# Circuitscape/Circuitscape.jl

Hardware: NVIDIA H100
Metric: pair_solves_per_sec (higher is better)
Workload: dtype f64

## Files before the change

circuitscape_b200/csrc/cs_b200.cu:

```cuda
#include "../../include/cs_b200.h"

#include <cuda_runtime.h>

#include <algorithm>
#include <chrono>
#include <cmath>
#include <cstdarg>
#include <cstdio>
#include <cstdlib>
#include <cstring>
#include <limits>
#include <string>
#include <type_traits>
#include <vector>

#include "amg_host.hpp"
#include "win_host.hpp"
#include "kernels.cuh"
#include "raster_assembly.cuh"
#include "setup_device.hpp"

using namespace csb;

namespace {
// ... 659 lines not shown
  if (rc) return rc;
  return cs_b200_reset_currents(h);
}

template <typename T>
int build_operators(cs_b200_handle* h, const csb_dev::HostPattern& hp, csb_dev::SeedJob* job,
                    const csb_dev::DeviceSeed* dseed) {
  int rc = CS_B200_OK;
  k_dinv<T><<<std::min<int64_t>((h->n_pad + 255) / 256, 4096), 256, 0, h->stream>>>(
      (int)h->n, (int)h->n_pad, h->d_rowptr, h->d_colidx, (const T*)h->d_vals, (T*)h->d_dinv);
  const bool want_win = h->opts.window >= 0 && (h->opts.window > 0 || h->n >= 20000) && (win_mask() & 1);
  const bool want_amg = h->opts.precond == CS_B200_PRECOND_AMG;
  Tick tick;
  if (want_win || h->opts.stencil > 0) {
    rc = device_stencil<T>(h, h->A0);
    if (!rc && !h->A0.dia && want_win) rc = device_windows<T>(h, h->A0, h->n_pad, (const T*)h->d_dinv);
    if (rc) { csb_dev::seed_discard(job); return rc; }
    tick(h->A0.dia ? "finest operator: stencil form" : "finest operator: windows");
  }
  if (want_amg) {
    rc = setup_amg_device<T>(h, hp, job, dseed);
    if (rc) return rc;
    if (h->amg && h->A0.dia && !h->P2) {
      const size_t pe = (size_t)h->n_pad * h->ktmax * sizeof(T);
      cudaError_t e = cudaMalloc(&h->P2, pe);
      if (e == cudaSuccess) e = cudaMemsetAsync(h->P2, 0, pe, h->stream);
      if (e != cudaSuccess) return set_err(h, CS_B200_ERR_CUDA, "CUDA error %s (second p panel)", cudaGetErrorString(e));
    }
  } else {
    csb_dev::seed_discard(job);
  }
  Tick tick1;
  csb_dev::trim_pool(h->device);
  tick1("scratch pool released");
  return CS_B200_OK;
}

int common_create(cs_b200_handle* h, const cs_b200_opts* opts) {
  if (opts) h->opts = *opts;
  if (h->opts.panel_width == 0) h->opts.panel_width = 8;
  if (h->opts.check_every <= 0) h->opts.check_every = 16;
  if (h->opts.resid_gate <= 0) h->opts.resid_gate = 1e-4;
  if (h->opts.use_graph == 0) h->opts.use_graph = 1;
  const int pw = h->opts.panel_width;
  if (pw != 1 && pw != 2 && pw != 4 && pw != 8)
    return set_err(h, CS_B200_ERR_ARG, "panel_width must be 1, 2, 4 or 8 (got %d)", pw);
  h->ktmax = pw;
  if (h->opts.precond != CS_B200_PRECOND_JACOBI && h->opts.precond != CS_B200_PRECOND_AMG)
    return set_err(h, CS_B200_ERR_UNSUPPORTED, "unknown preconditioner %d", h->opts.precond);
  int ndev = 0;
  cudaError_t e = cudaGetDeviceCount(&ndev);
  if (e != cudaSuccess || ndev == 0)
    return set_err(h, CS_B200_ERR_CUDA,
                   "no CUDA device available (%s): libcsb200 has no CPU fallback",
                   cudaGetErrorString(e));
  if (h->device < 0 || h->device >= ndev)
    return set_err(h, CS_B200_ERR_ARG, "device %d out of range (0..%d)", h->device, ndev - 1);
  CK(h, cudaSetDevice(h->device));
  cudaDeviceProp prop;
  CK(h, cudaGetDeviceProperties(&prop, h->device));
  h->num_sms = prop.multiProcessorCount;
  h->grid_spmm = h->num_sms * 8;
  h->grid_ew = h->num_sms * 4;
  CK(h, cudaStreamCreateWithFlags(&h->stream, cudaStreamNonBlocking));
  CK(h, cudaEventCreate(&h->ev0));
  CK(h, cudaEventCreate(&h->ev1));
  CK(h, cudaEventCreate(&h->ev2));
  CK(h, cudaEventCreate(&h->ev3));
  h->n_pad = (h->n + 3) / 4 * 4;
  return CS_B200_OK;
}

template <typename I>
void narrow_indices(const I* src, int64_t count, int base, std::vector<int>& dst) {
  dst.resize(count);
  for (int64_t i = 0; i < count; ++i) dst[i] = (int)(src[i] - base);
}

template <typename T>
CsrDev<T> view(const DevCsr& m) {
  return CsrDev<T>{m.rowptr, m.colidx, (const T*)m.vals, m.bstart, m.nblocks, m.nrows};
}

template <typename T, int KT, int MODE>
void launch_spmm_on(cs_b200_handle* h, const DevCsr& m, const T* X, T* Y, const T* B, const T* dinv,
                    double omega, bool timed) {
  const int grid = std::max(1, std::min(h->grid_spmm, m.nblocks));
  cudaEvent_t e0 = nullptr, e1 = nullptr;
  const bool prof = h->profile && timed;
  if (prof) {
    if (h->prof_used + 2 > h->prof_ev.size()) {
      for (int i = 0; i < 2; ++i) { cudaEvent_t e; cudaEventCreate(&e); h->prof_ev.push_back(e); }
    }
    e0 = h->prof_ev[h->prof_used++];
    e1 = h->prof_ev[h->prof_used++];
    double bytes = (double)m.nnz * (sizeof(T) + 4) + (double)(m.nrows + 1) * 4 +
                   2.0 * (double)m.nrows * KT * sizeof(T);
    if (MODE == SP_RESNORM || MODE == SP_RES || MODE == SP_JACOBI || MODE == SP_JACOBI_DOT)
      bytes += (double)m.nrows * KT * sizeof(T);
    if (MODE == SP_JACOBI || MODE == SP_JACOBI_DOT) bytes += (double)m.nrows * sizeof(T);
    h->prof_bytes += bytes;
    h->prof_slot.push_back(2 * MODE + (sizeof(T) == 4 ? 1 : 0));
    h->prof_pair_bytes.push_back(bytes);
    cudaEventRecord(e0, h->stream);
  }
  const SpmmEpi<T> ep{B, dinv, (T)omega, h->d_ctl, h->d_partials};
  if (m.dia && MODE != SP_ADD) {
    if constexpr (MODE != SP_ADD) {
      const DiaDev<T> a{(const T*)m.dia, m.dia_ld, m.nrows, m.dia_nr};
      constexpr int V16 = 16 / (int)sizeof(T);
      constexpr int CGn = KT / (KT < V16 ? KT : V16);
      const int rpp = NT / CGn;
      const long long ntiles = (long long)((m.dia_nr + rpp - 1) / rpp) *
                               ((((long long)m.nrows + m.dia_nr - 1) / m.dia_nr + ST_TC - 1) / ST_TC);
      const int sg = (int)std::max<long long>(1, std::min<long long>(h->grid_spmm, ntiles));
      k_stencil<T, KT, MODE><<<sg, NT, 0, h->stream>>>(a, X, Y, ep);
    }
  } else if (m.win_meta) {
    const WinCsr<T> w{m.win_meta, m.blob, m.has_dinv, m.rowptr, m.colidx, (const T*)m.vals, m.win_nblocks};
    if (m.lpr == 4) {
      constexpr int SMEM = WinSmem2<T, KT, MODE, true>::TOTAL;
      constexpr int SB = WinMap<T, KT, true>::SB;
      const int wg = std::max(1, std::min(h->num_sms, (m.win_nblocks + SB - 1) / SB));
      static bool once[64] = {};
      bool& set = once[h->device & 63];
      if (!set) { cudaFuncSetAttribute(k_spmm_win<T, KT, MODE, true>, cudaFuncAttributeMaxDynamicSharedMemorySize, SMEM); set = true; }
      k_spmm_win<T, KT, MODE, true><<<wg, WTT, SMEM, h->stream>>>(w, X, Y, ep);
    } else {
      constexpr int SMEM = WinSmem2<T, KT, MODE, false>::TOTAL;
      constexpr int SB = WinMap<T, KT, false>::SB;
      const int wg = std::max(1, std::min(h->num_sms, (m.win_nblocks + SB - 1) / SB));
      static bool once[64] = {};
      bool& set = once[h->device & 63];
      if (!set) { cudaFuncSetAttribute(k_spmm_win<T, KT, MODE, false>, cudaFuncAttributeMaxDynamicSharedMemorySize, SMEM); set = true; }
      k_spmm_win<T, KT, MODE, false><<<wg, WTT, SMEM, h->stream>>>(w, X, Y, ep);
    }
  } else if (m.lpr == 4 && KT * 4 <= 32) {
    k_spmm<T, KT, MODE, (KT * 4 <= 32 ? 4 : 1)><<<grid, NT, 0, h->stream>>>(view<T>(m), X, Y, ep);
  } else {
    k_spmm<T, KT, MODE, 1><<<grid, NT, 0, h->stream>>>(view<T>(m), X, Y, ep);
  }
  if (prof) cudaEventRecord(e1, h->stream);
  h->stats.kernel_launches++;
  if (timed) h->stats.spmm_launches++;
}

template <typename T, int KT, int MODE>
void launch_spmm(cs_b200_handle* h, const T* X, T* Y, const T* B) {
  launch_spmm_on<T, KT, MODE>(h, h->A0, X, Y, B, (const T*)h->d_dinv, 0.0, true);
}

void harvest_profile(cs_b200_handle* h) {
  for (size_t i = 0; i + 1 < h->prof_used; i += 2) {
    float ms = 0;
    if (cudaEventElapsedTime(&ms, h->prof_ev[i], h->prof_ev[i + 1]) == cudaSuccess) {
      h->prof_ms += ms;
      h->prof_launches++;
      if (i / 2 < h->prof_slot.size()) {
        const int sl = h->prof_slot[i / 2];
        h->prof_slot_ms[sl] += ms;
        h->prof_slot_bytes[sl] += h->prof_pair_bytes[i / 2];
        h->prof_slot_launches[sl]++;
      }
    }
  }
  h->prof_used = 0;
  h->prof_slot.clear();
  h->prof_pair_bytes.clear();
}

template <typename T, int KT>
int ew_grid(cs_b200_handle* h) {
  const size_t nelem = (size_t)h->n_pad * KT;
  const size_t per = (size_t)NT * Vec<T>::N;
  return (int)std::min<size_t>(h->grid_ew, (nelem + per - 1) / per);
}

template <typename T, int KT>
int ew_grid_n(cs_b200_handle* h, int64_t n_pad) {
  const size_t nelem = (size_t)n_pad * KT;
  const size_t per = (size_t)NT * Vec<T>::N;
  return (int)std::max<size_t>(1, std::min<size_t>(h->grid_ew, (nelem + per - 1) / per));
}

inline bool implicit_x0(const DevLevel& L) {
  static const bool off = std::getenv("CS_B200_NO_IMPLICIT_X0") != nullptr || std::getenv("CS_B200_NO_FUSED_PROLONG") != nullptr;
  return L.A.dia != nullptr && !off;
}

template <typename T, int KT>
void launch_stencil_res0(cs_b200_handle* h, DevLevel& L, const T* B, T* Tout, bool timed) {
  const DevCsr& m = L.A;
  const DiaDev<T> a{(const T*)m.dia, m.dia_ld, m.nrows, m.dia_nr};
  const SpmmEpi<T> ep{B, (const T*)L.dinv, (T)L.omega, h->d_ctl, h->d_partials};
  constexpr int V16 = 16 / (int)sizeof(T);
  constexpr int CGn = KT / (KT < V16 ? KT : V16);
  const int rpp = NT / CGn;
  const long long ntiles = (long long)((m.dia_nr + rpp - 1) / rpp) *
                           ((((long long)m.nrows + m.dia_nr - 1) / m.dia_nr + ST_TC - 1) / ST_TC);
  const int sg = (int)std::max<long long>(1, std::min<long long>(h->grid_spmm, ntiles));
  cudaEvent_t e0 = nullptr, e1 = nullptr;
  const bool prof = h->profile && timed;
  if (prof) {
    if (h->prof_used + 2 > h->prof_ev.size())
      for (int i = 0; i < 2; ++i) { cudaEvent_t e; cudaEventCreate(&e); h->prof_ev.push_back(e); }
    e0 = h->prof_ev[h->prof_used++];
    e1 = h->prof_ev[h->prof_used++];
    const double fb = (double)m.nnz * (sizeof(T) + 4) + (double)(m.nrows + 1) * 4 + 3.0 * (double)m.nrows * KT * sizeof(T);
    h->prof_bytes += fb;
    h->prof_slot.push_back(2 * (int)SP_RES + (sizeof(T) == 4 ? 1 : 0));
    h->prof_pair_bytes.push_back(fb);
    cudaEventRecord(e0, h->stream);
  }
  k_stencil<T, KT, SP_RES0><<<sg, NT, 0, h->stream>>>(a, nullptr, Tout, ep);
  if (prof) cudaEventRecord(e1, h->stream);
  h->stats.kernel_launches++;
  if (timed) h->stats.spmm_launches++;
}

template <typename T, int KT, int MODE>
void launch_prolong_jacobi(cs_b200_handle* h, DevLevel& L, const T* Yc, const T* X0, T* Yout, const T* B, bool timed) {
  const DevCsr& m = L.A;
  const DiaDev<T> a{(const T*)m.dia, m.dia_ld, m.nrows, m.dia_nr};
  const CsrP<T> p{L.P.rowptr, L.P.colidx, (const T*)L.P.vals, L.P.ell_col, (const T*)L.P.ell_val, L.P.ell_ld};
  const SpmmEpi<T> ep{B, (const T*)L.dinv, (T)L.omega, h->d_ctl, h->d_partials};
  using S = PjShape<T, KT>;
  constexpr int SMEM = S::SMEM;
  constexpr int MINB = sizeof(T) == 4 ? PJ_MINB_F32 : PJ_MINB_F64;
  static_assert(SMEM <= 48 * 1024, "the strip buffers fit the default dynamic shared memory");
  int occ = 0;
  cudaOccupancyMaxActiveBlocksPerMultiprocessor(&occ, k_stencil_prolong_jacobi<T, KT, MODE, MINB>, NT, SMEM);
  occ = std::max(1, occ);
  const long long nsteps = (long long)((m.dia_nr + S::RPS - 1) / S::RPS) *
                           (((long long)m.nrows + m.dia_nr - 1) / m.dia_nr);
  const int grid = (int)std::max<long long>(1, std::min<long long>(std::min(h->grid_spmm, h->num_sms * occ), nsteps));
  cudaEvent_t e0 = nullptr, e1 = nullptr;
  const bool prof = h->profile && timed;
  if (prof) {
    if (h->prof_used + 2 > h->prof_ev.size())
      for (int i = 0; i < 2; ++i) { cudaEvent_t e; cudaEventCreate(&e); h->prof_ev.push_back(e); }
    e0 = h->prof_ev[h->prof_used++];
    e1 = h->prof_ev[h->prof_used++];
    const double fb = (double)m.nnz * (sizeof(T) + 4) + (double)(m.nrows + 1) * 4 + 3.0 * (double)m.nrows * KT * sizeof(T) +
                      (double)m.nrows * sizeof(T) + (double)L.P.nnz * (sizeof(T) + 4) + (double)(m.nrows + 1) * 4 +
                      2.0 * (double)m.nrows * KT * sizeof(T);
    h->prof_bytes += fb;
    h->prof_slot.push_back(2 * 7 + (sizeof(T) == 4 ? 1 : 0));
    h->prof_pair_bytes.push_back(fb);
    cudaEventRecord(e0, h->stream);
  }
  k_stencil_prolong_jacobi<T, KT, MODE, MINB><<<grid, NT, SMEM, h->stream>>>(a, p, Yc, X0, Yout, ep);
  if (prof) cudaEventRecord(e1, h->stream);
  h->stats.kernel_launches++;
  if (timed) h->stats.spmm_launches++;
}

struct VcBufs { void *b0, *x0, *t0, *y0; };

template <typename T, int KT>
void launch_vcycle_on(cs_b200_handle* h, std::vector<DevLevel>& lv, const VcBufs& vb, bool level0_presmoothed) {
  const int nl = (int)lv.size();
  auto B = [&](int l) { return l == 0 ? (T*)vb.b0 : (T*)lv[l].b; };
  auto X = [&](int l) { return l == 0 ? (T*)vb.x0 : (T*)lv[l].x; };
  auto Tm = [&](int l) { return l == 0 ? (T*)vb.t0 : (T*)lv[l].t; };
  auto Y = [&](int l) { return l == 0 ? (T*)vb.y0 : (T*)lv[l].y; };
  for (int l = 0; l < nl - 1; ++l) {
    DevLevel& L = lv[l];
    const size_t nelem = (size_t)L.n_pad * KT;
    if (implicit_x0(L)) {
      launch_stencil_res0<T, KT>(h, L, B(l), Tm(l), l == 0);
    } else {
      if (!(l == 0 && level0_presmoothed)) {
        k_jacobi0<T, KT><<<ew_grid_n<T, KT>(h, L.n_pad), NT, 0, h->stream>>>(
            nelem, B(l), (const T*)L.dinv, (T)L.omega, X(l));
        h->stats.kernel_launches++;
      }
      launch_spmm_on<T, KT, SP_RES>(h, L.A, X(l), Tm(l), B(l), nullptr, 0.0, l == 0);
    }
    launch_spmm_on<T, KT, SP_PLAIN>(h, L.R, Tm(l), B(l + 1), nullptr, nullptr, 0.0, false);
  }
  {
    DevLevel& C = lv[nl - 1];
    if (h->d_pinv) {
      k_coarse_dense<T, KT><<<((int)C.n * KT + NT - 1) / NT, NT, 0, h->stream>>>((int)C.n, h->d_pinv, (const T*)B(nl - 1), Y(nl - 1));
      h->stats.kernel_launches++;
    } else {
      const int l = nl - 1;
      k_jacobi0<T, KT><<<ew_grid_n<T, KT>(h, C.n_pad), NT, 0, h->stream>>>(
          (size_t)C.n_pad * KT, B(l), (const T*)C.dinv, (T)C.omega, X(l));
      h->stats.kernel_launches++;
      launch_spmm_on<T, KT, SP_JACOBI>(h, C.A, X(l), Y(l), B(l), (const T*)C.dinv, C.omega, false);
      launch_spmm_on<T, KT, SP_JACOBI>(h, C.A, Y(l), X(l), B(l), (const T*)C.dinv, C.omega, false);
      launch_spmm_on<T, KT, SP_JACOBI>(h, C.A, X(l), Y(l), B(l), (const T*)C.dinv, C.omega, false);
    }
  }
  static const bool fuse_off = std::getenv("CS_B200_NO_FUSED_PROLONG") != nullptr;
  for (int l = nl - 2; l >= 0; --l) {
    DevLevel& L = lv[l];
    if (L.A.dia && !fuse_off) {
      const T* x0 = implicit_x0(L) ? nullptr : X(l);
      if (l == 0) launch_prolong_jacobi<T, KT, SP_JACOBI_DOT>(h, L, Y(l + 1), x0, Y(l), B(l), true);
      else launch_prolong_jacobi<T, KT, SP_JACOBI>(h, L, Y(l + 1), x0, Y(l), B(l), false);
      continue;
    }
    launch_spmm_on<T, KT, SP_ADD>(h, L.P, Y(l + 1), X(l), X(l) , nullptr, 0.0, false);
    if (l == 0)
      launch_spmm_on<T, KT, SP_JACOBI_DOT>(h, L.A, X(l), Y(l), B(l), (const T*)L.dinv, L.omega, true);
    else
      launch_spmm_on<T, KT, SP_JACOBI>(h, L.A, X(l), Y(l), B(l), (const T*)L.dinv, L.omega, false);
  }
}

template <typename T, int KT>
void launch_vcycle(cs_b200_handle* h, bool level0_presmoothed) {
  if (h->mixed) {
    const VcBufs vb{h->R32, h->X32, h->T32, h->Z32};
    launch_vcycle_on<float, KT>(h, h->lv32, vb, level0_presmoothed);
  } else {
    const VcBufs vb{h->R, h->stage, h->AP, h->Z};
    launch_vcycle_on<T, KT>(h, h->lv, vb, level0_presmoothed);
  }
}

template <typename T, int KT>
void launch_seg_set(cs_b200_handle* h, void* panel, int set_b_only, T v) {
  k_seg_set<T, KT><<<2 * KT, NT, 0, h->stream>>>((T*)panel, h->d_rg_seg, h->d_rg_rows, set_b_only, v);
  h->stats.kernel_launches++;
}

template <typename T, int KT>
void mask_z(cs_b200_handle* h) {
  if (!h->rg_on) return;
  if (h->mixed) launch_seg_set<float, KT>(h, h->Z32, 0, 0.0f);
  else launch_seg_set<T, KT>(h, h->Z, 0, T(0));
}

inline GraphSlot& graph_slot(cs_b200_handle* h, int kt) {
  return (h->rg_on ? h->rgraphs : h->graphs)[kt_index(kt)];
}

void drop_graphs(GraphSlot* slots) {
  for (int i = 0; i < 4; ++i) {
    if (slots[i].exec) cudaGraphExecDestroy(slots[i].exec);
    if (slots[i].loop_exec) cudaGraphExecDestroy(slots[i].loop_exec);
    slots[i] = GraphSlot{};
  }
}

inline bool fused_cg(const cs_b200_handle* h) {
  static const bool off = std::getenv("CS_B200_NO_FUSED_CG") != nullptr;
  return h->amg && h->A0.dia && h->P2 && !off;
}

template <typename T, int KT, typename TV>
void launch_stencil_cg(cs_b200_handle* h, const TV* Z) {
  const DevCsr& m = h->A0;
  const DiaDev<T> a{(const T*)m.dia, m.dia_ld, m.nrows, m.dia_nr};
  constexpr int V16 = 16 / (int)sizeof(T);
  constexpr int CGn = KT / (KT < V16 ? KT : V16);
  const int rpp = NT / CGn;
  const long long ntiles = (long long)((m.dia_nr + rpp - 1) / rpp) *
                           ((((long long)m.nrows + m.dia_nr - 1) / m.dia_nr + ST_TC - 1) / ST_TC);
  const int sg = (int)std::max<long long>(1, std::min<long long>(h->grid_spmm, ntiles));
  cudaEvent_t e0 = nullptr, e1 = nullptr;
  if (h->profile) {
    if (h->prof_used + 2 > h->prof_ev.size())
      for (int i = 0; i < 2; ++i) { cudaEvent_t e; cudaEventCreate(&e); h->prof_ev.push_back(e); }
    e0 = h->prof_ev[h->prof_used++];
    e1 = h->prof_ev[h->prof_used++];
    const double pe = (double)m.nrows * KT * sizeof(T);
    const double fb = (double)m.nrows * 9 * sizeof(T) + (double)m.nrows * KT * sizeof(TV) + 3.0 * pe + 1.5 * pe;
    h->prof_bytes += fb;
    h->prof_slot.push_back(2 * PROF_CGF + (sizeof(T) == 4 ? 1 : 0));
    h->prof_pair_bytes.push_back(fb);
    cudaEventRecord(e0, h->stream);
  }
  k_stencil_cg<T, KT, TV><<<sg, NT, 0, h->stream>>>(a, Z, (T*)h->P2, (T*)h->P, (T*)h->X, (T*)h->AP, h->d_ctl,
                                                     h->d_partials);
  if (h->profile) cudaEventRecord(e1, h->stream);
  h->stats.kernel_launches++;
  h->stats.spmm_launches++;
}

template <typename T, int KT>
void launch_iteration(cs_b200_handle* h) {
  const size_t nelem = (size_t)h->n_pad * KT;
  const int g = ew_grid<T, KT>(h);
  const bool fused = fused_cg(h);
  if (fused) {
    if (h->mixed) launch_stencil_cg<T, KT, float>(h, (const float*)h->Z32);
    else launch_stencil_cg<T, KT, T>(h, (const T*)h->Z);
  } else {
    launch_spmm<T, KT, SP_CG>(h, (const T*)h->P, (T*)h->AP, nullptr);
  }
  if (h->rg_on) launch_seg_set<T, KT>(h, h->AP, 0, T(0));
  if (!h->amg) {
    k_cg_update_r<T, KT><<<g, NT, 0, h->stream>>>(nelem, (const T*)h->AP, (const T*)h->d_dinv,
                                                  (T*)h->R, h->d_ctl, h->d_partials);
    k_cg_update_xp<T, KT><<<g, NT, 0, h->stream>>>(nelem, (const T*)h->R, (const T*)h->d_dinv,
                                                   (T*)h->X, (T*)h->P, h->d_ctl);
    h->stats.kernel_launches += 2;
  } else {
    if (h->mixed) {
      k_cg_update_r0<T, KT, float><<<g, NT, 0, h->stream>>>(nelem, (const T*)h->AP, (const T*)h->d_dinv,
                                                            (T)h->lv[0].omega, (T*)h->R,
                                                            implicit_x0(h->lv32[0]) ? nullptr : (float*)h->X32,
                                                            (float*)h->R32, h->d_ctl);
      launch_vcycle<T, KT>(h, true);
      mask_z<T, KT>(h);
      if (!fused)
        k_cg_update_xp2<T, KT, float><<<g, NT, 0, h->stream>>>(nelem, (const float*)h->Z32, (T*)h->X, (T*)h->P,
                                                               h->d_ctl);
    } else {
      k_cg_update_r0<T, KT, T><<<g, NT, 0, h->stream>>>(nelem, (const T*)h->AP, (const T*)h->d_dinv,
                                                        (T)h->lv[0].omega, (T*)h->R,
                                                        implicit_x0(h->lv[0]) ? nullptr : (T*)h->stage, nullptr,
                                                        h->d_ctl);
      launch_vcycle<T, KT>(h, true);
      mask_z<T, KT>(h);
      if (!fused)
        k_cg_update_xp2<T, KT, T><<<g, NT, 0, h->stream>>>(nelem, (const T*)h->Z, (T*)h->X, (T*)h->P, h->d_ctl);
    }
    h->stats.kernel_launches += fused ? 1 : 2;
  }
}

template <typename T, int KT>
void finish_x(cs_b200_handle* h) {
  if (!fused_cg(h)) return;
  k_cg_x_tail<T, KT><<<ew_grid<T, KT>(h), NT, 0, h->stream>>>((size_t)h->n_pad * KT, (const T*)h->P2, (const T*)h->P,
                                                             (T*)h->X, h->d_ctl);
  h->stats.kernel_launches++;
}

template <typename T, int KT>
int run_chunk(cs_b200_handle* h, int chunk) {
  GraphSlot& gs = graph_slot(h, KT);
  if (h->opts.use_graph > 0 && !h->profile) {
    if (!gs.exec || gs.chunk != chunk) {
      if (gs.exec) cudaGraphExecDestroy(gs.exec);
      gs.exec = nullptr;
      cudaGraph_t graph;
      const int64_t kl = h->stats.kernel_launches, sl = h->stats.spmm_launches;
      CK(h, cudaStreamBeginCapture(h->stream, cudaStreamCaptureModeThreadLocal));
      for (int i = 0; i < chunk; ++i) launch_iteration<T, KT>(h);
      CK(h, cudaStreamEndCapture(h->stream, &graph));
      gs.kernels = h->stats.kernel_launches - kl;
      gs.spmms = h->stats.spmm_launches - sl;
      h->stats.kernel_launches = kl;
      h->stats.spmm_launches = sl;
      CK(h, cudaGraphInstantiate(&gs.exec, graph, 0));
      cudaGraphDestroy(graph);
      gs.chunk = chunk;
    }
    CK(h, cudaGraphLaunch(gs.exec, h->stream));
    h->stats.kernel_launches += gs.kernels;
    h->stats.spmm_launches += gs.spmms;
  } else {
    for (int i = 0; i < chunk; ++i) launch_iteration<T, KT>(h);
    CK(h, cudaGetLastError());
  }
// ... 1904 lines not shown
```

circuitscape_b200/csrc/kernels.cuh:

```cuda
#pragma once
#include <cuda_runtime.h>
#include <stdint.h>

namespace csb {

constexpr int NT = 256;
constexpr int NWARP = NT / 32;
constexpr int NNZ_CAP = 2304;
constexpr int MAXKT = 8;

struct PanelCtl {
  double rho[MAXKT];
  double pap[MAXKT];
  double alpha[MAXKT];
  double beta[MAXKT];
  double tol[MAXKT];
  double rho0[MAXKT];
  double resid[MAXKT];
  double bnorm[MAXKT];
  double xsrc[MAXKT];
  double xdst[MAXKT];
  double maxpos[MAXKT];
  double maxneg[MAXKT];
  double weight[MAXKT];
// ... 947 lines not shown
    a2[i] = (T)ctl->alpha_ring[(it + 1) % 3][c0 + i];
  }
  double dot0[CPT];
#pragma unroll
  for (int i = 0; i < CPT; ++i) dot0[i] = 0.0;

  for (long long t = blockIdx.x; t < ntiles; t += gridDim.x) {
    const int tc = (int)(t / nrc), rc = (int)(t % nrc);
    const int r = rc * RPP + rl;
    if (r >= nr) continue;
    const int cend = min(ncol, (tc + 1) * ST_TC);
    for (int c = tc * ST_TC; c < cend; ++c) {
      const long long row_l = (long long)c * nr + r;
      if (row_l >= n) break;
      const int row = (int)row_l;
      T v[9];
#pragma unroll
      for (int s = 0; s < 9; ++s) v[s] = __ldcs(A.vals + (size_t)s * A.ld + row);
      TV zv[9][CPT];
      T pv[9][CPT];
#pragma unroll
      for (int s = 0; s < 9; ++s) {
        int j = row + (s / 3 - 1) * nr + (s % 3 - 1);
        j = max(0, min(n - 1, j));
        ldvec<TV, CPT>(Z + (size_t)j * KT + c0, zv[s]);
        ldvec<T, CPT, true>(Pold + (size_t)j * KT + c0, pv[s]);
      }
      const size_t o = (size_t)row * KT + c0;
      T xo[CPT], pd[CPT], po[CPT];
      if (pair) {
        ldvec<T, CPT>(X + o, xo);
        ldvec<T, CPT>(Pd + o, pd);
      }
#pragma unroll
      for (int i = 0; i < CPT; ++i) po[i] = pv[4][i];
#pragma unroll
      for (int s = 0; s < 9; ++s)
#pragma unroll
        for (int i = 0; i < CPT; ++i) pv[s][i] = (T)zv[s][i] + be[i] * pv[s][i];
      T acc[CPT];
#pragma unroll
      for (int i = 0; i < CPT; ++i) acc[i] = T(0);
#pragma unroll
      for (int s = 0; s < 9; ++s)
#pragma unroll
        for (int i = 0; i < CPT; ++i) acc[i] += v[s] * pv[s][i];
#pragma unroll
      for (int i = 0; i < CPT; ++i) dot0[i] += (double)acc[i] * (double)pv[4][i];
      stvec<T, CPT>(Y + o, acc);
      stvec<T, CPT>(Pd + o, pv[4]);
      if (pair) {
#pragma unroll
        for (int i = 0; i < CPT; ++i) {
          xo[i] += a2[i] * pd[i];
          xo[i] += a1[i] * po[i];
        }
        stvec<T, CPT>(X + o, xo);
      }
    }
  }
  CSB_REDUCE_SMEM(1, KT)
  double v[1][CPT];
#pragma unroll
  for (int i = 0; i < CPT; ++i) v[0][i] = dot0[i];
  if (grid_reduce<KT, CPT, 1, false>(v, partials, &ctl->ticket, s_warp, s_tree, s_out)) {
    if (tid < KT) {
      const double pap = s_out[tid];
      const double al = (ctl->active[tid] && pap > 0.0) ? ctl->rho[tid] / pap : 0.0;
      ctl->pap[tid] = pap;
      ctl->alpha[tid] = al;
      ctl->alpha_ring[it % 3][tid] = al;
    }
  }
}

template <typename T, int KT, typename TV>
__global__ void __launch_bounds__(NT, CGF_MINB)
k_stencil_cg(const DiaDev<T> A, const TV* __restrict__ Z, T* Pb0, T* Pb1, T* __restrict__ X, T* __restrict__ Y,
             PanelCtl* ctl, double* partials) {
  const int it = ctl->iter;
  stencil_cg_body<T, KT, TV>(A, Z, (it & 1) ? Pb0 : Pb1, (it & 1) ? Pb1 : Pb0, X, Y, ctl, partials, it);
}

constexpr int PJ_RING = 4;
constexpr int PJ_MINB_F32 = 3;
constexpr int PJ_MINB_F64 = 2;

template <typename T> struct CsrP {
  const int* rowptr;
  const int* colidx;
  const T* vals;
  const int* ell_col;
  const T* ell_val;
  size_t ell_ld;
};

template <typename T, int KT> struct PjShape {
  static constexpr int V16 = 16 / (int)sizeof(T);
  static constexpr int CPT = KT < V16 ? KT : V16;
  static constexpr int CG = KT / CPT;
  static constexpr int RH = NT / CG;
  static constexpr int RPS = RH - 2;
  static constexpr bool VSMEM = sizeof(T) == 4;
  static constexpr int SMEM = (PJ_RING * RH * KT + 2 * NT * CPT + 2 * NT + (VSMEM ? 2 * 9 * RH : 0)) * (int)sizeof(T);
};

template <typename T, int KT, int MODE, int MINB>
__global__ void __launch_bounds__(NT, MINB)
k_stencil_prolong_jacobi(const DiaDev<T> A, const CsrP<T> P, const T* __restrict__ Yc, const T* __restrict__ X0,
                         T* __restrict__ Z, const SpmmEpi<T> ep) {
  static_assert(MODE == SP_JACOBI || MODE == SP_JACOBI_DOT, "post-smoothing modes only");
  using S = PjShape<T, KT>;
  constexpr int CPT = S::CPT, CG = S::CG, RH = S::RH, RPS = S::RPS;
  extern __shared__ __align__(16) unsigned char pj_smem[];
  T* xs = reinterpret_cast<T*>(pj_smem);
  T* bsm = xs + PJ_RING * RH * KT;
  T* wsm = bsm + 2 * NT * CPT;
  T* vsm = wsm + 2 * NT;
  const int tid = threadIdx.x;
  const int g = tid % CG, rr = tid / CG, c0 = g * CPT;
  const bool inner = rr >= 1 && rr <= RPS;
  const int n = A.n, nr = A.nr;
  const int ncol = (n + nr - 1) / nr;
  const int nstrip = (nr + RPS - 1) / RPS;
  const int nstep = nstrip * ncol;
  const int per = (nstep + (int)gridDim.x - 1) / (int)gridDim.x;
  const int s_beg = (int)min((long long)nstep, (long long)blockIdx.x * per);
  const int s_end = (int)min((long long)nstep, ((long long)blockIdx.x + 1) * per);
  const bool ell = P.ell_col != nullptr;
  double dot0[CPT];
#pragma unroll
  for (int i = 0; i < CPT; ++i) dot0[i] = 0.0;

  for (int s0 = s_beg; s0 < s_end;) {
    const int strip = s0 / ncol, cb = s0 % ncol;
    const int ce = min(ncol, cb + (s_end - s0));
    s0 += ce - cb;
    const int r = strip * RPS + rr - 1;
    const bool rok = r >= 0 && r < nr;
    auto row_of = [&](int c, int& row) {
      const long long rl = (long long)c * nr + r;
      const bool ok = rok && c >= 0 && c < ncol && rl < n;
      row = ok ? (int)rl : 0;
      return ok;
    };
    auto ell_row = [&](int row, int (&cj)[4], T (&pv)[4]) {
#pragma unroll
      for (int q = 0; q < 4; ++q) {
        cj[q] = __ldg(P.ell_col + (size_t)q * P.ell_ld + row);
        pv[q] = __ldg(P.ell_val + (size_t)q * P.ell_ld + row);
      }
    };
    int rowc, rowp = 0;
    bool okc = row_of(cb - 1, rowc), okp = false;
    int cj[4] = {0, 0, 0, 0};
    T pv[4] = {T(0), T(0), T(0), T(0)};
    if (ell) ell_row(rowc, cj, pv);
    __syncthreads();
    for (int c = cb - 1; c <= ce; ++c) {
      const int rel = c - (cb - 1);
      const bool zdo = inner && c > cb && okp;
      T v[9];
      if constexpr (S::VSMEM) {
        if (zdo && g == 0) {
#pragma unroll
          for (int s = 0; s < 9; ++s)
// ... 803 lines not shown
```

profiles/run_iteration_breakdown.py:

```python
#!/usr/bin/env python
import argparse
import ctypes as C
import json
import os
import re
import subprocess
import sys
from collections import defaultdict

sys.path.insert(0, os.path.dirname(os.path.dirname(os.path.abspath(__file__))))
import numpy as np

PEAK_GBS = 3350.0
KT = 8


def card():
    try:
        out = subprocess.run(["nvidia-smi", "--query-gpu=name,power.limit", "--format=csv,noheader"],
                             capture_output=True, text=True, timeout=30).stdout.strip().splitlines()
        name, pl = [s.strip() for s in out[0].split(",")]
        return {"name": name, "power_limit": pl}
    except Exception as e:
        return {"name": None, "power_limit": None, "error": str(e)}


def level_dims(f):
    out = []
    for l in range(64):
        lev = {}
        for name, which in (("A", 0), ("P", 1), ("R", 2)):
            nr, nc, nnz = C.c_int64(), C.c_int64(), C.c_int64()
            om, win = C.c_double(), C.c_int()
            rc = f._lib.cs_b200_level_info(f._h, l, which, C.byref(nr), C.byref(nc), C.byref(nnz),
                                           C.byref(om), C.byref(win))
            lev[name] = (nr.value, nc.value, nnz.value, win.value) if rc == 0 else None
        if lev["A"] is None:
            break
        out.append(lev)
    return out


def short(name):
    name = name.replace("(anonymous namespace)::", "").replace("csb::", "")
    name = re.sub(r"^void ", "", name)
    depth, cut = 0, len(name)
    for i, ch in enumerate(name):
        if ch == "<":
            depth += 1
        elif ch == ">":
            depth -= 1
        elif ch == "(" and depth == 0:
            cut = i
            break
    return name[:cut].replace(" ", "")


def finest_bytes(levels, prolong_form):
    n = levels[0]["A"][0]
    n1 = levels[1]["A"][0] if len(levels) > 1 else 0
    nnz_r = levels[0]["R"][2] if levels[0]["R"] else 0
    d64, d32 = 8 * KT, 4 * KT
    rps = 256 // 2 - 2
    if prolong_form == "tile":
        halo = (130 * 10) / (128 * 8)
        prol = n * (halo * (d32 + 4 + 32 + d32) + 9 * 4 + d32 + 4 + d32)
    else:
        halo = (rps + 2) / rps
        prol = n * (halo * (d32 + 4 + 32 + d32) + 9 * 4 + d32)
    return {
        "k_stencil<double,8,1>": n * (9 * 8 + d64 + d64),
        "k_stencil_cg<double,8,float>": n * (9 * 8 + d32 + 3 * d64 + 1.5 * d64),
        "k_cg_update_r0<double,8,float>": n * (d64 + 8 + 2 * d64 + d32),
        "k_stencil<float,8,7>": n * (9 * 4 + d32 + 4 + d32),
        "k_spmm_win<float,8,0,*>#1": nnz_r * 6 + n1 * 2 + n * d32 + n1 * d32,
        "k_stencil_prolong_jacobi<float,8,5,*>": prol,
        "k_cg_update_xp2<double,8,float>": n * (d32 + 4 * d64),
    }, {"n": n, "n1": n1, "nnz_R0": nnz_r, "prolong_halo_factor": halo}


def match_bytes(key, table):
    for pat, b in table.items():
        base, _, occ = pat.partition("#")
        rx = "^" + re.escape(base).replace(r"\*", r"[^,>]+") + "$"
        name, _, slot = key.partition("#")
        if re.match(rx, name) and (not occ or (slot or "1").split("/")[0] == occ):
            return b
    return None


def main():
    ap = argparse.ArgumentParser()
    ap.add_argument("--rows", type=int, default=3163)
    ap.add_argument("--reps", type=int, default=20)
    ap.add_argument("--prolong-form", default="strip", choices=["strip", "tile"])
    ap.add_argument("--out", default="")
    a = ap.parse_args()

    import torch
    from torch.profiler import ProfilerActivity, profile
    import circuitscape_b200 as cb
    from circuitscape_b200 import graph
    if not torch.cuda.is_available():
        raise SystemExit("needs a CUDA device")
    L, _ = graph.synthetic_raster_laplacian(a.rows, a.rows, seed=42)
    with cb.construct_cholesky_factor(L, cb.CUDASolver()) as f:
        levels = level_dims(f)
        f.bench_cg_iter(KT, reps=5)
        ms_iter = f.bench_cg_iter(KT, reps=a.reps)
        torch.cuda.synchronize()
        with profile(activities=[ProfilerActivity.CUDA]) as prof:
            f.bench_cg_iter(KT, reps=a.reps)
            torch.cuda.synchronize()
    evs = [e for e in prof.events() if e.device_type.name == "CUDA" and "memcpy" not in e.name.lower()
           and "memset" not in e.name.lower()]
    evs.sort(key=lambda e: e.time_range.start)
    starts = [i for i, e in enumerate(evs) if short(e.name).startswith(("k_stencil<double,8,1>", "k_stencil_cg<double,8,",
                                                                        "k_spmm_win<double,8,1,"))]
    iters = [evs[starts[j]:starts[j + 1]] for j in range(len(starts) - 1)]
    iters = iters[3:] if len(iters) > a.reps else iters
    if len(starts) > 1:
        last = evs[starts[-1]:]
        iters.append(last[:len(iters[0])] if iters else last)
    agg = defaultdict(lambda: [0, 0.0])
    for it in iters:
        names = [short(e.name) for e in it]
        tot = defaultdict(int)
        for nm in names:
            tot[nm] += 1
        seen = defaultdict(int)
        for e, nm in zip(it, names):
            seen[nm] += 1
            key = nm if tot[nm] == 1 else f"{nm}#{seen[nm]}/{tot[nm]}"
            agg[key][0] += 1
            agg[key][1] += e.time_range.elapsed_us()
    niter = max(1, len(iters))
    table, shape = finest_bytes(levels, a.prolong_form)
    sum_us = sum(v[1] for v in agg.values()) / niter
    rows = {}
    for key, (cnt, us) in sorted(agg.items(), key=lambda kv: -kv[1][1]):
        avg = us / cnt
        r = {"launches_per_iter": cnt / niter, "avg_us": avg, "share": (us / niter) / sum_us}
        b = match_bytes(key, table)
        if b is not None:
            r.update({"bytes": b, "GB/s": b / (avg * 1e-6) / 1e9, "frac_of_peak": b / (avg * 1e-6) / 1e9 / PEAK_GBS})
        rows[key] = r
    res = {"card": card(), "rows": a.rows, "k": KT, "iterations_profiled": niter,
           "iter_ms_events": ms_iter, "iter_ms_kernel_sum": sum_us / 1e3, "peak_GBs": PEAK_GBS,
           "peak_source": "H100 SXM data sheet (HBM3)", "prolong_form": a.prolong_form, "shape": shape,
           "levels": [{k: v for k, v in lev.items()} for lev in levels], "kernels": rows}
    line = json.dumps(res)
    print(line)
    if a.out:
        os.makedirs(os.path.dirname(os.path.abspath(a.out)), exist_ok=True)
        with open(a.out, "w") as fh:
            fh.write(line + "\n")


if __name__ == "__main__":
    main()
```

Measured before the change: 127.2.

## Add cp.async multi-stage pipelined stencil and fused CG stencil kernels

```diff
diff --git a/circuitscape_b200/csrc/cs_b200.cu b/circuitscape_b200/csrc/cs_b200.cu
--- a/circuitscape_b200/csrc/cs_b200.cu
+++ b/circuitscape_b200/csrc/cs_b200.cu
@@ -765,6 +765,24 @@
   return CsrDev<T>{m.rowptr, m.colidx, (const T*)m.vals, m.bstart, m.nblocks, m.nrows};
 }
 
+inline bool stencil_pipe() {
+  static const bool off = std::getenv("CS_B200_NO_STENCIL_PIPE") != nullptr;
+  return !off;
+}
+
+template <typename T, int KT, int MODE>
+void launch_stencil(cs_b200_handle* h, const DiaDev<T>& a, const T* X, T* Y, const SpmmEpi<T>& ep, int sg) {
+  if (!stencil_pipe()) {
+    k_stencil<T, KT, MODE><<<sg, NT, 0, h->stream>>>(a, X, Y, ep);
+    return;
+  }
+  constexpr int SMEM = StPipe<T, KT, MODE>::D::BYTES;
+  static bool once[64] = {};
+  bool& set = once[h->device & 63];
+  if (!set) { cudaFuncSetAttribute(k_stencil_pipe<T, KT, MODE>, cudaFuncAttributeMaxDynamicSharedMemorySize, SMEM); set = true; }
+  k_stencil_pipe<T, KT, MODE><<<sg, NT, SMEM, h->stream>>>(a, X, Y, ep);
+}
+
 template <typename T, int KT, int MODE>
 void launch_spmm_on(cs_b200_handle* h, const DevCsr& m, const T* X, T* Y, const T* B, const T* dinv,
                     double omega, bool timed) {
@@ -797,7 +815,7 @@
       const long long ntiles = (long long)((m.dia_nr + rpp - 1) / rpp) *
                                ((((long long)m.nrows + m.dia_nr - 1) / m.dia_nr + ST_TC - 1) / ST_TC);
       const int sg = (int)std::max<long long>(1, std::min<long long>(h->grid_spmm, ntiles));
-      k_stencil<T, KT, MODE><<<sg, NT, 0, h->stream>>>(a, X, Y, ep);
+      launch_stencil<T, KT, MODE>(h, a, X, Y, ep, sg);
     }
   } else if (m.win_meta) {
     const WinCsr<T> w{m.win_meta, m.blob, m.has_dinv, m.rowptr, m.colidx, (const T*)m.vals, m.win_nblocks};
@@ -895,7 +913,7 @@
     h->prof_pair_bytes.push_back(fb);
     cudaEventRecord(e0, h->stream);
   }
-  k_stencil<T, KT, SP_RES0><<<sg, NT, 0, h->stream>>>(a, nullptr, Tout, ep);
+  launch_stencil<T, KT, SP_RES0>(h, a, nullptr, Tout, ep, sg);
   if (prof) cudaEventRecord(e1, h->stream);
   h->stats.kernel_launches++;
   if (timed) h->stats.spmm_launches++;
@@ -1058,8 +1076,17 @@
     h->prof_pair_bytes.push_back(fb);
     cudaEventRecord(e0, h->stream);
   }
-  k_stencil_cg<T, KT, TV><<<sg, NT, 0, h->stream>>>(a, Z, (T*)h->P2, (T*)h->P, (T*)h->X, (T*)h->AP, h->d_ctl,
-                                                     h->d_partials);
+  if (stencil_pipe()) {
+    constexpr int SMEM = StPipeCg<T, KT, TV>::D::BYTES;
+    static bool once[64] = {};
+    bool& set = once[h->device & 63];
+    if (!set) { cudaFuncSetAttribute(k_stencil_cg_pipe<T, KT, TV>, cudaFuncAttributeMaxDynamicSharedMemorySize, SMEM); set = true; }
+    k_stencil_cg_pipe<T, KT, TV><<<sg, NT, SMEM, h->stream>>>(a, Z, (T*)h->P2, (T*)h->P, (T*)h->X, (T*)h->AP,
+                                                              h->d_ctl, h->d_partials);
+  } else {
+    k_stencil_cg<T, KT, TV><<<sg, NT, 0, h->stream>>>(a, Z, (T*)h->P2, (T*)h->P, (T*)h->X, (T*)h->AP, h->d_ctl,
+                                                       h->d_partials);
+  }
   if (h->profile) cudaEventRecord(e1, h->stream);
   h->stats.kernel_launches++;
   h->stats.spmm_launches++;
diff --git a/circuitscape_b200/csrc/kernels.cuh b/circuitscape_b200/csrc/kernels.cuh
--- a/circuitscape_b200/csrc/kernels.cuh
+++ b/circuitscape_b200/csrc/kernels.cuh
@@ -1053,6 +1053,381 @@
   stencil_cg_body<T, KT, TV>(A, Z, (it & 1) ? Pb0 : Pb1, (it & 1) ? Pb1 : Pb0, X, Y, ctl, partials, it);
 }
 
+constexpr int ST_SMAX = 4;
+constexpr int st_a16(int b) { return (b + 15) & ~15; }
+
+template <int PANEL, int OWN, int MINB> struct StDepth {
+  static constexpr int BUDGET = 228 * 1024 / MINB - 1024 - 3 * 1024;
+  static constexpr int FIT = (BUDGET - 3 * PANEL - OWN) / (PANEL + OWN);
+  static constexpr int S = FIT < 1 ? 1 : (FIT > ST_SMAX ? ST_SMAX : FIT);
+  static constexpr int BYTES = (S + 3) * PANEL + (S + 1) * OWN;
+};
+
+template <int B>
+__device__ __forceinline__ void cp_async_zfill(void* dst, const void* src, bool ok) {
+  const int sz = ok ? B : 0;
+  if constexpr (B == 16)
+    asm volatile("cp.async.cg.shared.global [%0], [%1], 16, %2;" ::"r"(smem_u32(dst)), "l"(src), "r"(sz) : "memory");
+  else
+    asm volatile("cp.async.ca.shared.global [%0], [%1], %2, %3;" ::"r"(smem_u32(dst)), "l"(src), "n"(B), "r"(sz)
+                 : "memory");
+}
+__device__ __forceinline__ void cp_async_commit() { asm volatile("cp.async.commit_group;" ::: "memory"); }
+template <int N> __device__ __forceinline__ void cp_async_wait() {
+  asm volatile("cp.async.wait_group %0;" ::"n"(N) : "memory");
+}
+
+template <typename U, int W, int NROWS>
+__device__ __forceinline__ void cp_rows(U* dst, const U* src, long long g0, int n) {
+  constexpr int RB = W * (int)sizeof(U);
+  constexpr int CH = RB < 16 ? RB : 16;
+  constexpr int CPR = RB / CH;
+  constexpr int NCH = NROWS * CPR;
+#pragma unroll 1
+  for (int q0 = 0; q0 < NCH; q0 += NT) {
+    const int q = q0 + (int)threadIdx.x;
+    if (NCH % NT == 0 || q < NCH) {
+      const long long g = g0 + q / CPR;
+      const bool ok = g >= 0 && g < n;
+      cp_async_zfill<CH>(reinterpret_cast<char*>(dst) + q * CH,
+                         reinterpret_cast<const char*>(src + (ok ? g : 0) * W) + (q % CPR) * CH, ok);
+    }
+  }
+}
+
+template <typename T, int RPP>
+__device__ __forceinline__ void cp_diag(T* dst, const DiaDev<T>& A, long long row0) {
+  constexpr int NCH = 9 * RPP;
+#pragma unroll 1
+  for (int q0 = 0; q0 < NCH; q0 += NT) {
+    const int q = q0 + (int)threadIdx.x;
+    if (NCH % NT == 0 || q < NCH) {
+      const long long g = row0 + q % RPP;
+      const bool ok = g < A.n;
+      cp_async_zfill<(int)sizeof(T)>(dst + q, A.vals + (size_t)(q / RPP) * A.ld + (ok ? g : 0), ok);
+    }
+  }
+}
+
+struct StStep {
+  long long t;
+  int cs, ce, c, r0;
+  __device__ __forceinline__ void start(long long t_, int nrc, int ncol, int rpp) {
+    t = t_;
+    r0 = (int)(t % nrc) * rpp;
+    cs = (int)(t / nrc) * ST_TC;
+    ce = min(ncol, cs + ST_TC);
+    c = cs - 1;
+  }
+  __device__ __forceinline__ void next(int nrc, int ncol, int rpp) {
+    if (++c > ce) start(t + gridDim.x, nrc, ncol, rpp);
+  }
+};
+
+template <int S, int RPP, class Issue, class Compute>
+__device__ __forceinline__ void stencil_pipe(int n, int nr, Issue&& issue, Compute&& compute) {
+  constexpr int RP = S + 3, RO = S + 1;
+  const int ncol = (n + nr - 1) / nr;
+  const int nrc = (nr + RPP - 1) / RPP;
+  const long long ntiles = (long long)nrc * ((ncol + ST_TC - 1) / ST_TC);
+  StStep ld, st;
+  ld.start(blockIdx.x, nrc, ncol, RPP);
+  st = ld;
+  int lp = 0, lo = 0, sp = 0, so = 0;
+#pragma unroll 1
+  for (int k = 0; k < S; ++k) {
+    if (ld.t < ntiles) issue(ld, lp, lo);
+    cp_async_commit();
+    ld.next(nrc, ncol, RPP);
+    lp = lp + 1 == RP ? 0 : lp + 1;
+    lo = lo + 1 == RO ? 0 : lo + 1;
+  }
+#pragma unroll 1
+  while (st.t < ntiles) {
+    cp_async_wait<S - 1>();
+    __syncthreads();
+    if (ld.t < ntiles) issue(ld, lp, lo);
+    cp_async_commit();
+    ld.next(nrc, ncol, RPP);
+    lp = lp + 1 == RP ? 0 : lp + 1;
+    lo = lo + 1 == RO ? 0 : lo + 1;
+    if (st.c > st.cs) compute(st, sp, so);
+    st.next(nrc, ncol, RPP);
+    sp = sp + 1 == RP ? 0 : sp + 1;
+    so = so + 1 == RO ? 0 : so + 1;
+  }
+  cp_async_wait<0>();
+}
+
+template <typename T, int KT, int MODE> struct StPipe {
+  static constexpr int V16 = 16 / (int)sizeof(T);
+  static constexpr int CPT = KT < V16 ? KT : V16;
+  static constexpr int RPP = NT / (KT / CPT);
+  static constexpr bool NEEDB = (MODE == SP_RESNORM || MODE == SP_RES || MODE == SP_JACOBI || MODE == SP_JACOBI_DOT);
+  static constexpr bool NEEDD = (MODE == SP_JACOBI || MODE == SP_JACOBI_DOT);
+  static constexpr int PX = st_a16((RPP + 2) * KT * (int)sizeof(T));
+  static constexpr int PANEL = PX + (MODE == SP_RES0 ? st_a16((RPP + 2) * (int)sizeof(T)) : 0);
+  static constexpr int OD = st_a16(9 * RPP * (int)sizeof(T));
+  static constexpr int OB = NEEDB ? st_a16(RPP * KT * (int)sizeof(T)) : 0;
+  static constexpr int OWN = OD + OB + (NEEDD ? st_a16(RPP * (int)sizeof(T)) : 0);
+  using D = StDepth<PANEL, OWN, 3>;
+};
+
+template <typename T, int KT, int MODE>
+__global__ void __launch_bounds__(NT, 3)
+k_stencil_pipe(const DiaDev<T> A, const T* __restrict__ X, T* __restrict__ Y, const SpmmEpi<T> ep) {
+  using SP = StPipe<T, KT, MODE>;
+  constexpr int CPT = SP::CPT, RPP = SP::RPP, S = SP::D::S;
+  constexpr int RP = S + 3;
+  extern __shared__ __align__(128) unsigned char st_sm[];
+  unsigned char* const pring = st_sm;
+  unsigned char* const oring = st_sm + RP * SP::PANEL;
+  const int tid = threadIdx.x;
+  const int cg = tid % (KT / CPT), rl = tid / (KT / CPT), c0 = cg * CPT;
+  const int n = A.n, nr = A.nr;
+  double dot0[CPT], dot1[CPT];
+#pragma unroll
+  for (int i = 0; i < CPT; ++i) dot0[i] = dot1[i] = 0.0;
+
+  const T* const G = MODE == SP_RES0 ? ep.B : X;
+  auto issue = [&](const StStep& s, int lp, int lo) {
+    unsigned char* ps = pring + lp * SP::PANEL;
+    const long long g0 = (long long)s.c * nr + s.r0 - 1;
+    cp_rows<T, KT, RPP + 2>(reinterpret_cast<T*>(ps), G, g0, n);
+    if (MODE == SP_RES0) cp_rows<T, 1, RPP + 2>(reinterpret_cast<T*>(ps + SP::PX), ep.dinv, g0, n);
+    if (s.c > s.cs) {
+      unsigned char* os = oring + lo * SP::OWN;
+      const long long row0 = (long long)(s.c - 1) * nr + s.r0;
+      cp_diag<T, RPP>(reinterpret_cast<T*>(os), A, row0);
+      if (SP::NEEDB) cp_rows<T, KT, RPP>(reinterpret_cast<T*>(os + SP::OD), ep.B, row0, n);
+      if (SP::NEEDD) cp_rows<T, 1, RPP>(reinterpret_cast<T*>(os + SP::OD + SP::OB), ep.dinv, row0, n);
+    }
+  };
+  auto compute = [&](const StStep& s, int sp, int so) {
+    const int c = s.c - 1, r = s.r0 + rl;
+    const long long row_l = (long long)c * nr + r;
+    if (r >= nr || row_l >= n) return;
+    const int row = (int)row_l;
+    const T* xs[3];
+    const T* ws[3];
+#pragma unroll
+    for (int d = 0; d < 3; ++d) {
+      const int k = sp + d + RP - 2;
+      const unsigned char* p = pring + (k >= RP ? k - RP : k) * SP::PANEL;
+      xs[d] = reinterpret_cast<const T*>(p);
+      ws[d] = reinterpret_cast<const T*>(p + SP::PX);
+    }
+    const unsigned char* os = oring + so * SP::OWN;
+    const T* dg = reinterpret_cast<const T*>(os);
+    T acc[CPT], xo[CPT];
+#pragma unroll
+    for (int i = 0; i < CPT; ++i) acc[i] = T(0);
+#pragma unroll
+    for (int s9 = 0; s9 < 9; ++s9) {
+      T xv[CPT];
+      ldvec<T, CPT>(xs[s9 / 3] + (rl + s9 % 3) * KT + c0, xv);
+      if (s9 == 4) {
+#pragma unroll
+        for (int i = 0; i < CPT; ++i) xo[i] = xv[i];
+      }
+      const T vs = MODE == SP_RES0 ? dg[s9 * RPP + rl] * (ep.omega * ws[s9 / 3][rl + s9 % 3]) : dg[s9 * RPP + rl];
+#pragma unroll
+      for (int i = 0; i < CPT; ++i) acc[i] += vs * xv[i];
+    }
+    const size_t o = (size_t)row * KT + c0;
+    T out[CPT], bb[CPT];
+    if (SP::NEEDB) ldvec<T, CPT>(reinterpret_cast<const T*>(os + SP::OD) + rl * KT + c0, bb);
+    T dv = T(0);
+    if (SP::NEEDD) dv = ep.omega * reinterpret_cast<const T*>(os + SP::OD + SP::OB)[rl];
+#pragma unroll
+    for (int i = 0; i < CPT; ++i) {
+      if (MODE == SP_PLAIN) {
+        out[i] = acc[i];
+      } else if (MODE == SP_CG) {
+        out[i] = acc[i];
+        dot0[i] += (double)acc[i] * (double)xo[i];
+      } else if (MODE == SP_RESNORM) {
+        const T rr = bb[i] - acc[i];
+        out[i] = rr;
+        dot0[i] += (double)rr * (double)rr;
+        dot1[i] += (double)bb[i] * (double)bb[i];
+      } else if (MODE == SP_RES) {
+        out[i] = bb[i] - acc[i];
+      } else if (MODE == SP_RES0) {
+        out[i] = xo[i] - acc[i];
+      } else {
+        const T yn = xo[i] + dv * (bb[i] - acc[i]);
+        out[i] = yn;
+        if (MODE == SP_JACOBI_DOT) dot0[i] += (double)bb[i] * (double)yn;
+      }
+    }
+    stvec<T, CPT>(Y + o, out);
+  };
+  stencil_pipe<S, RPP>(n, nr, issue, compute);
+
+  if (MODE == SP_CG) {
+    CSB_REDUCE_SMEM(1, KT)
+    double v[1][CPT];
+#pragma unroll
+    for (int i = 0; i < CPT; ++i) v[0][i] = dot0[i];
+    if (grid_reduce<KT, CPT, 1, false>(v, ep.partials, &ep.ctl->ticket, s_warp, s_tree, s_out)) {
+      if (tid < KT) {
+        const double pap = s_out[tid];
+        ep.ctl->pap[tid] = pap;
+        ep.ctl->alpha[tid] = (ep.ctl->active[tid] && pap > 0.0) ? ep.ctl->rho[tid] / pap : 0.0;
+      }
+    }
+  } else if (MODE == SP_RESNORM) {
+    CSB_REDUCE_SMEM(2, KT)
+    double v[2][CPT];
+#pragma unroll
+    for (int i = 0; i < CPT; ++i) { v[0][i] = dot0[i]; v[1][i] = dot1[i]; }
+    if (grid_reduce<KT, CPT, 2, false>(v, ep.partials, &ep.ctl->ticket, s_warp, s_tree, s_out)) {
+      if (tid < KT) {
+        ep.ctl->resid[tid] = s_out[tid];
+        ep.ctl->bnorm[tid] = s_out[KT + tid];
+      }
+    }
+  } else if (MODE == SP_JACOBI_DOT) {
+    CSB_REDUCE_SMEM(1, KT)
+    double v[1][CPT];
+#pragma unroll
+    for (int i = 0; i < CPT; ++i) v[0][i] = dot0[i];
+    if (grid_reduce<KT, CPT, 1, false>(v, ep.partials, &ep.ctl->ticket, s_warp, s_tree, s_out))
+      cg_after_precond<KT>(ep.ctl, s_out);
+  }
+}
+
+constexpr int CGP_MINB = 3;
+
+template <typename T, int KT, typename TV> struct StPipeCg {
+  static constexpr int V16 = 16 / (int)sizeof(T);
+  static constexpr int CPT = KT < V16 ? KT : V16;
+  static constexpr int RPP = NT / (KT / CPT);
+  static constexpr int PP = st_a16((RPP + 2) * KT * (int)sizeof(T));
+  static constexpr int PANEL = PP + st_a16((RPP + 2) * KT * (int)sizeof(TV));
+  static constexpr int OD = st_a16(9 * RPP * (int)sizeof(T));
+  static constexpr int OX = st_a16(RPP * KT * (int)sizeof(T));
+  static constexpr int OWN = OD + 2 * OX;
+  using D = StDepth<PANEL, OWN, CGP_MINB>;
+};
+
+template <typename T, int KT, typename TV>
+__global__ void __launch_bounds__(NT, CGP_MINB)
+k_stencil_cg_pipe(const DiaDev<T> A, const TV* __restrict__ Z, T* Pb0, T* Pb1, T* __restrict__ X, T* __restrict__ Y,
+                  PanelCtl* ctl, double* partials) {
+  using SP = StPipeCg<T, KT, TV>;
+  constexpr int CPT = SP::CPT, RPP = SP::RPP, S = SP::D::S;
+  constexpr int RP = S + 3;
+  extern __shared__ __align__(128) unsigned char st_sm[];
+  unsigned char* const pring = st_sm;
+  unsigned char* const oring = st_sm + RP * SP::PANEL;
+  const int it = ctl->iter;
+  const T* const Pold = (it & 1) ? Pb0 : Pb1;
+  T* const Pd = (it & 1) ? Pb1 : Pb0;
+  const int tid = threadIdx.x;
+  const int cg = tid % (KT / CPT), rl = tid / (KT / CPT), c0 = cg * CPT;
+  const int n = A.n, nr = A.nr;
+  const bool pair = it & 1;
+  T be[CPT], a1[CPT], a2[CPT];
+#pragma unroll
+  for (int i = 0; i < CPT; ++i) {
+    be[i] = (T)ctl->beta[c0 + i];
+    a1[i] = (T)ctl->alpha_ring[(it + 2) % 3][c0 + i];
+    a2[i] = (T)ctl->alpha_ring[(it + 1) % 3][c0 + i];
+  }
+  double dot0[CPT];
+#pragma unroll
+  for (int i = 0; i < CPT; ++i) dot0[i] = 0.0;
+
+  auto issue = [&](const StStep& s, int lp, int lo) {
+    unsigned char* ps = pring + lp * SP::PANEL;
+    const long long g0 = (long long)s.c * nr + s.r0 - 1;
+    cp_rows<T, KT, RPP + 2>(reinterpret_cast<T*>(ps), Pold, g0, n);
+    cp_rows<TV, KT, RPP + 2>(reinterpret_cast<TV*>(ps + SP::PP), Z, g0, n);
+    if (s.c > s.cs) {
+      unsigned char* os = oring + lo * SP::OWN;
+      const long long row0 = (long long)(s.c - 1) * nr + s.r0;
+      cp_diag<T, RPP>(reinterpret_cast<T*>(os), A, row0);
+      if (pair) {
+        cp_rows<T, KT, RPP>(reinterpret_cast<T*>(os + SP::OD), X, row0, n);
+        cp_rows<T, KT, RPP>(reinterpret_cast<T*>(os + SP::OD + SP::OX), Pd, row0, n);
+      }
+    }
+  };
+  auto compute = [&](const StStep& s, int sp, int so) {
+    const int c = s.c - 1, r = s.r0 + rl;
+    const long long row_l = (long long)c * nr + r;
+    if (r >= nr || row_l >= n) return;
+    const int row = (int)row_l;
+    const T* ps[3];
+    const TV* zs[3];
+#pragma unroll
+    for (int d = 0; d < 3; ++d) {
+      const int k = sp + d + RP - 2;
+      const unsigned char* p = pring + (k >= RP ? k - RP : k) * SP::PANEL;
+      ps[d] = reinterpret_cast<const T*>(p);
+      zs[d] = reinterpret_cast<const TV*>(p + SP::PP);
+    }
+    const unsigned char* os = oring + so * SP::OWN;
+    const T* dg = reinterpret_cast<const T*>(os);
+    T acc[CPT], po[CPT], pc[CPT];
+#pragma unroll
+    for (int i = 0; i < CPT; ++i) acc[i] = T(0);
+#pragma unroll
+    for (int s9 = 0; s9 < 9; ++s9) {
+      T pv[CPT];
+      TV zv[CPT];
+      ldvec<T, CPT>(ps[s9 / 3] + (rl + s9 % 3) * KT + c0, pv);
+      ldvec<TV, CPT>(zs[s9 / 3] + (rl + s9 % 3) * KT + c0, zv);
+      if (s9 == 4) {
+#pragma unroll
+        for (int i = 0; i < CPT; ++i) po[i] = pv[i];
+      }
+#pragma unroll
+      for (int i = 0; i < CPT; ++i) pv[i] = (T)zv[i] + be[i] * pv[i];
+      if (s9 == 4) {
+#pragma unroll
+        for (int i = 0; i < CPT; ++i) pc[i] = pv[i];
+      }
+      const T vs = dg[s9 * RPP + rl];
+#pragma unroll
+      for (int i = 0; i < CPT; ++i) acc[i] += vs * pv[i];
+    }
+#pragma unroll
+    for (int i = 0; i < CPT; ++i) dot0[i] += (double)acc[i] * (double)pc[i];
+    const size_t o = (size_t)row * KT + c0;
+    stvec<T, CPT>(Y + o, acc);
+    stvec<T, CPT>(Pd + o, pc);
+    if (pair) {
+      T xo[CPT], pd[CPT];
+      ldvec<T, CPT>(reinterpret_cast<const T*>(os + SP::OD) + rl * KT + c0, xo);
+      ldvec<T, CPT>(reinterpret_cast<const T*>(os + SP::OD + SP::OX) + rl * KT + c0, pd);
+#pragma unroll
+      for (int i = 0; i < CPT; ++i) {
+        xo[i] += a2[i] * pd[i];
+        xo[i] += a1[i] * po[i];
+      }
+      stvec<T, CPT>(X + o, xo);
+    }
+  };
+  stencil_pipe<S, RPP>(n, nr, issue, compute);
+
+  CSB_REDUCE_SMEM(1, KT)
+  double v[1][CPT];
+#pragma unroll
+  for (int i = 0; i < CPT; ++i) v[0][i] = dot0[i];
+  if (grid_reduce<KT, CPT, 1, false>(v, partials, &ctl->ticket, s_warp, s_tree, s_out)) {
+    if (tid < KT) {
+      const double pap = s_out[tid];
+      const double al = (ctl->active[tid] && pap > 0.0) ? ctl->rho[tid] / pap : 0.0;
+      ctl->pap[tid] = pap;
+      ctl->alpha[tid] = al;
+      ctl->alpha_ring[it % 3][tid] = al;
+    }
+  }
+}
+
 constexpr int PJ_RING = 4;
 constexpr int PJ_MINB_F32 = 3;
 constexpr int PJ_MINB_F64 = 2;
diff --git a/profiles/run_iteration_breakdown.py b/profiles/run_iteration_breakdown.py
--- a/profiles/run_iteration_breakdown.py
+++ b/profiles/run_iteration_breakdown.py
@@ -68,11 +68,16 @@
     else:
         halo = (rps + 2) / rps
         prol = n * (halo * (d32 + 4 + 32 + d32) + 9 * 4 + d32)
+    cg_step = n * (9 * 8 + d32 + 3 * d64 + 1.5 * d64)
+    res0 = n * (9 * 4 + d32 + 4 + d32)
     return {
         "k_stencil<double,8,1>": n * (9 * 8 + d64 + d64),
-        "k_stencil_cg<double,8,float>": n * (9 * 8 + d32 + 3 * d64 + 1.5 * d64),
+        "k_stencil_pipe<double,8,1>": n * (9 * 8 + d64 + d64),
+        "k_stencil_cg<double,8,float>": cg_step,
+        "k_stencil_cg_pipe<double,8,float>": cg_step,
         "k_cg_update_r0<double,8,float>": n * (d64 + 8 + 2 * d64 + d32),
-        "k_stencil<float,8,7>": n * (9 * 4 + d32 + 4 + d32),
+        "k_stencil<float,8,7>": res0,
+        "k_stencil_pipe<float,8,7>": res0,
         "k_spmm_win<float,8,0,*>#1": nnz_r * 6 + n1 * 2 + n * d32 + n1 * d32,
         "k_stencil_prolong_jacobi<float,8,5,*>": prol,
         "k_cg_update_xp2<double,8,float>": n * (d32 + 4 * d64),
@@ -116,6 +121,8 @@
            and "memset" not in e.name.lower()]
     evs.sort(key=lambda e: e.time_range.start)
     starts = [i for i, e in enumerate(evs) if short(e.name).startswith(("k_stencil<double,8,1>", "k_stencil_cg<double,8,",
+                                                                        "k_stencil_pipe<double,8,1>",
+                                                                        "k_stencil_cg_pipe<double,8,",
                                                                         "k_spmm_win<double,8,1,"))]
     iters = [evs[starts[j]:starts[j + 1]] for j in range(len(starts) - 1)]
     iters = iters[3:] if len(iters) > a.reps else iters
```

Measured after the change: 135.6 (median of 6 runs). +6.6%, better.
